# mit-han-lab/duo-attention

Measured on NVIDIA H100. Metric: decode tok/s @512K ctx (+ prefill tok/s @128K in `prefill`), Llama-3-8B, DuoAttention 50% retrieval heads, higher is better.
Workload: dtype bf16

## Files before the change

duo_attention_b200/csrc/attn_tc.cu:

```cuda
#include <cstdlib>

#include "duo_common.cuh"

namespace duo {

constexpr int TC_THREADS = 384;
constexpr int TC_TILE = 128;
constexpr int TC_BOX_BYTES = TC_TILE * 128;
constexpr int TC_TILE_BYTES = 2 * TC_BOX_BYTES;
constexpr int TC_MAX_W = 2048;
constexpr int TC_SMEM_BYTES = 5 * TC_TILE_BYTES + TC_MAX_W + 1024;

struct TcParams {
  void* out;
  long long out_batch_stride;
  int q_len, n_q_heads, group, n_full, n_stream, batch;
  int sink, recent, W;
  long long full_len, total, lo;
  float scale_log2;
  int cache_scan;
  int n_tok_tiles;
  int seq_rank, seq_world, seq_block;
  float* part_o;
  float* part_lse;
};

__device__ __forceinline__ void wg_fence() { asm volatile("wgmma.fence.sync.aligned;" ::: "memory"); }
__device__ __forceinline__ void wg_commit() { asm volatile("wgmma.commit_group.sync.aligned;" ::: "memory"); }
template <int N>
__device__ __forceinline__ void wg_wait() {
  asm volatile("wgmma.wait_group.sync.aligned %0;" ::"n"(N) : "memory");
}
__device__ __forceinline__ void wg_fence_regs(float (&d)[64]) {
#pragma unroll
  for (int i = 0; i < 64; ++i) asm volatile("" : "+f"(d[i])::"memory");
}

__device__ __forceinline__ uint64_t make_smem_desc(uint32_t saddr, uint32_t lbo_bytes, uint32_t sbo_bytes) {
  uint64_t d = 0;
  d |= (uint64_t)((saddr >> 4) & 0x3FFF);
  d |= (uint64_t)((lbo_bytes >> 4) & 0x3FFF) << 16;
  d |= (uint64_t)((sbo_bytes >> 4) & 0x3FFF) << 32;
  d |= 1ull << 62;
  return d;
}

template <bool BF16>
__device__ __forceinline__ void wgmma_ss(float (&d)[64], uint64_t adesc, uint64_t bdesc, uint32_t accum) {
  if constexpr (BF16) {
    asm volatile(
        "{\n\t.reg .pred p;\n\tsetp.ne.b32 p, %66, 0;\n\t"
        "wgmma.mma_async.sync.aligned.m64n128k16.f32.bf16.bf16 {%0,%1,%2,%3,%4,%5,%6,%7,%8,%9,%10,%11,%12,%13,%14,%15,%16,%17,%18,%19,%20,%21,%22,%23,%24,%25,%26,%27,%28,%29,%30,%31,%32,%33,%34,%35,%36,%37,%38,%39,%40,%41,%42,%43,%44,%45,%46,%47,%48,%49,%50,%51,%52,%53,%54,%55,%56,%57,%58,%59,%60,%61,%62,%63}, %64, %65, p, 1, 1, 0, 0;\n\t}"
        : "+f"(d[0]), "+f"(d[1]), "+f"(d[2]), "+f"(d[3]), "+f"(d[4]), "+f"(d[5]), "+f"(d[6]), "+f"(d[7]), "+f"(d[8]), "+f"(d[9]), "+f"(d[10]), "+f"(d[11]), "+f"(d[12]), "+f"(d[13]), "+f"(d[14]), "+f"(d[15]), "+f"(d[16]), "+f"(d[17]), "+f"(d[18]), "+f"(d[19]), "+f"(d[20]), "+f"(d[21]), "+f"(d[22]), "+f"(d[23]), "+f"(d[24]), "+f"(d[25]), "+f"(d[26]), "+f"(d[27]), "+f"(d[28]), "+f"(d[29]), "+f"(d[30]), "+f"(d[31]), "+f"(d[32]), "+f"(d[33]), "+f"(d[34]), "+f"(d[35]), "+f"(d[36]), "+f"(d[37]), "+f"(d[38]), "+f"(d[39]), "+f"(d[40]), "+f"(d[41]), "+f"(d[42]), "+f"(d[43]), "+f"(d[44]), "+f"(d[45]), "+f"(d[46]), "+f"(d[47]), "+f"(d[48]), "+f"(d[49]), "+f"(d[50]), "+f"(d[51]), "+f"(d[52]), "+f"(d[53]), "+f"(d[54]), "+f"(d[55]), "+f"(d[56]), "+f"(d[57]), "+f"(d[58]), "+f"(d[59]), "+f"(d[60]), "+f"(d[61]), "+f"(d[62]), "+f"(d[63])
        : "l"(adesc), "l"(bdesc), "r"(accum));
  } else {
    asm volatile(
        "{\n\t.reg .pred p;\n\tsetp.ne.b32 p, %66, 0;\n\t"
        "wgmma.mma_async.sync.aligned.m64n128k16.f32.f16.f16 {%0,%1,%2,%3,%4,%5,%6,%7,%8,%9,%10,%11,%12,%13,%14,%15,%16,%17,%18,%19,%20,%21,%22,%23,%24,%25,%26,%27,%28,%29,%30,%31,%32,%33,%34,%35,%36,%37,%38,%39,%40,%41,%42,%43,%44,%45,%46,%47,%48,%49,%50,%51,%52,%53,%54,%55,%56,%57,%58,%59,%60,%61,%62,%63}, %64, %65, p, 1, 1, 0, 0;\n\t}"
        : "+f"(d[0]), "+f"(d[1]), "+f"(d[2]), "+f"(d[3]), "+f"(d[4]), "+f"(d[5]), "+f"(d[6]), "+f"(d[7]), "+f"(d[8]), "+f"(d[9]), "+f"(d[10]), "+f"(d[11]), "+f"(d[12]), "+f"(d[13]), "+f"(d[14]), "+f"(d[15]), "+f"(d[16]), "+f"(d[17]), "+f"(d[18]), "+f"(d[19]), "+f"(d[20]), "+f"(d[21]), "+f"(d[22]), "+f"(d[23]), "+f"(d[24]), "+f"(d[25]), "+f"(d[26]), "+f"(d[27]), "+f"(d[28]), "+f"(d[29]), "+f"(d[30]), "+f"(d[31]), "+f"(d[32]), "+f"(d[33]), "+f"(d[34]), "+f"(d[35]), "+f"(d[36]), "+f"(d[37]), "+f"(d[38]), "+f"(d[39]), "+f"(d[40]), "+f"(d[41]), "+f"(d[42]), "+f"(d[43]), "+f"(d[44]), "+f"(d[45]), "+f"(d[46]), "+f"(d[47]), "+f"(d[48]), "+f"(d[49]), "+f"(d[50]), "+f"(d[51]), "+f"(d[52]), "+f"(d[53]), "+f"(d[54]), "+f"(d[55]), "+f"(d[56]), "+f"(d[57]), "+f"(d[58]), "+f"(d[59]), "+f"(d[60]), "+f"(d[61]), "+f"(d[62]), "+f"(d[63])
        : "l"(adesc), "l"(bdesc), "r"(accum));
  }
}
template <bool BF16>
__device__ __forceinline__ void wgmma_rs(float (&d)[64], const uint32_t* a, uint64_t bdesc) {
  if constexpr (BF16) {
    asm volatile(
        "{\n\t.reg .pred p;\n\tsetp.ne.b32 p, %69, 0;\n\t"
        "wgmma.mma_async.sync.aligned.m64n128k16.f32.bf16.bf16 {%0,%1,%2,%3,%4,%5,%6,%7,%8,%9,%10,%11,%12,%13,%14,%15,%16,%17,%18,%19,%20,%21,%22,%23,%24,%25,%26,%27,%28,%29,%30,%31,%32,%33,%34,%35,%36,%37,%38,%39,%40,%41,%42,%43,%44,%45,%46,%47,%48,%49,%50,%51,%52,%53,%54,%55,%56,%57,%58,%59,%60,%61,%62,%63}, {%64, %65, %66, %67}, %68, p, 1, 1, 1;\n\t}"
        : "+f"(d[0]), "+f"(d[1]), "+f"(d[2]), "+f"(d[3]), "+f"(d[4]), "+f"(d[5]), "+f"(d[6]), "+f"(d[7]), "+f"(d[8]), "+f"(d[9]), "+f"(d[10]), "+f"(d[11]), "+f"(d[12]), "+f"(d[13]), "+f"(d[14]), "+f"(d[15]), "+f"(d[16]), "+f"(d[17]), "+f"(d[18]), "+f"(d[19]), "+f"(d[20]), "+f"(d[21]), "+f"(d[22]), "+f"(d[23]), "+f"(d[24]), "+f"(d[25]), "+f"(d[26]), "+f"(d[27]), "+f"(d[28]), "+f"(d[29]), "+f"(d[30]), "+f"(d[31]), "+f"(d[32]), "+f"(d[33]), "+f"(d[34]), "+f"(d[35]), "+f"(d[36]), "+f"(d[37]), "+f"(d[38]), "+f"(d[39]), "+f"(d[40]), "+f"(d[41]), "+f"(d[42]), "+f"(d[43]), "+f"(d[44]), "+f"(d[45]), "+f"(d[46]), "+f"(d[47]), "+f"(d[48]), "+f"(d[49]), "+f"(d[50]), "+f"(d[51]), "+f"(d[52]), "+f"(d[53]), "+f"(d[54]), "+f"(d[55]), "+f"(d[56]), "+f"(d[57]), "+f"(d[58]), "+f"(d[59]), "+f"(d[60]), "+f"(d[61]), "+f"(d[62]), "+f"(d[63])
        : "r"(a[0]), "r"(a[1]), "r"(a[2]), "r"(a[3]), "l"(bdesc), "r"(1));
  } else {
    asm volatile(
        "{\n\t.reg .pred p;\n\tsetp.ne.b32 p, %69, 0;\n\t"
        "wgmma.mma_async.sync.aligned.m64n128k16.f32.f16.f16 {%0,%1,%2,%3,%4,%5,%6,%7,%8,%9,%10,%11,%12,%13,%14,%15,%16,%17,%18,%19,%20,%21,%22,%23,%24,%25,%26,%27,%28,%29,%30,%31,%32,%33,%34,%35,%36,%37,%38,%39,%40,%41,%42,%43,%44,%45,%46,%47,%48,%49,%50,%51,%52,%53,%54,%55,%56,%57,%58,%59,%60,%61,%62,%63}, {%64, %65, %66, %67}, %68, p, 1, 1, 1;\n\t}"
        : "+f"(d[0]), "+f"(d[1]), "+f"(d[2]), "+f"(d[3]), "+f"(d[4]), "+f"(d[5]), "+f"(d[6]), "+f"(d[7]), "+f"(d[8]), "+f"(d[9]), "+f"(d[10]), "+f"(d[11]), "+f"(d[12]), "+f"(d[13]), "+f"(d[14]), "+f"(d[15]), "+f"(d[16]), "+f"(d[17]), "+f"(d[18]), "+f"(d[19]), "+f"(d[20]), "+f"(d[21]), "+f"(d[22]), "+f"(d[23]), "+f"(d[24]), "+f"(d[25]), "+f"(d[26]), "+f"(d[27]), "+f"(d[28]), "+f"(d[29]), "+f"(d[30]), "+f"(d[31]), "+f"(d[32]), "+f"(d[33]), "+f"(d[34]), "+f"(d[35]), "+f"(d[36]), "+f"(d[37]), "+f"(d[38]), "+f"(d[39]), "+f"(d[40]), "+f"(d[41]), "+f"(d[42]), "+f"(d[43]), "+f"(d[44]), "+f"(d[45]), "+f"(d[46]), "+f"(d[47]), "+f"(d[48]), "+f"(d[49]), "+f"(d[50]), "+f"(d[51]), "+f"(d[52]), "+f"(d[53]), "+f"(d[54]), "+f"(d[55]), "+f"(d[56]), "+f"(d[57]), "+f"(d[58]), "+f"(d[59]), "+f"(d[60]), "+f"(d[61]), "+f"(d[62]), "+f"(d[63])
        : "r"(a[0]), "r"(a[1]), "r"(a[2]), "r"(a[3]), "l"(bdesc), "r"(1));
  }
}

template <typename T>
struct TcType;
template <>
struct TcType<__nv_bfloat16> {
  static constexpr bool bf16 = true;
  __device__ static uint32_t pack(float a, float b) {
    __nv_bfloat162 v = __floats2bfloat162_rn(a, b);
    return *reinterpret_cast<uint32_t*>(&v);
  }
};
template <>
struct TcType<__half> {
  static constexpr bool bf16 = false;
  __device__ static uint32_t pack(float a, float b) {
    __half2 v = __floats2half2_rn(a, b);
    return *reinterpret_cast<uint32_t*>(&v);
  }
};

struct TcBarriers {
  uint64_t q_full;
  uint64_t k_full[2], k_empty[2], v_full[2], v_empty[2];
};

template <typename T, bool SEQ = false, bool SHARE = false>
__global__ void __launch_bounds__(TC_THREADS, 1)
duo_attn_tc_kernel(const __grid_constant__ CUtensorMap map_q, const __grid_constant__ CUtensorMap map_fk,
                   const __grid_constant__ CUtensorMap map_fv, const __grid_constant__ CUtensorMap map_rk,
                   const __grid_constant__ CUtensorMap map_rv, const TcParams p,
                   const __grid_constant__ CUtensorMap map_pk, const __grid_constant__ CUtensorMap map_pv,
                   const long long share_len) {
  static_assert(!(SEQ && SHARE), "a shared prefix is not sequence-sharded");
  extern __shared__ __align__(1024) uint8_t smem_raw[];
  uint8_t* smem = reinterpret_cast<uint8_t*>((reinterpret_cast<uintptr_t>(smem_raw) + 1023) & ~uintptr_t(1023));
  __shared__ TcBarriers bars;

  uint8_t* sQ = smem;
  uint8_t* sK = smem + 1 * TC_TILE_BYTES;
  uint8_t* sV = smem + 3 * TC_TILE_BYTES;
  uint8_t* sValid = smem + 5 * TC_TILE_BYTES;

  const int tid = threadIdx.x;
  const int b = blockIdx.y;

  int x = blockIdx.x;
  const int per_kvh = p.group * p.n_tok_tiles;
  const int kvh = x / per_kvh;
  x -= kvh * per_kvh;
  const int qh = kvh * p.group + x / p.n_tok_tiles;
  const int tok0 = (p.n_tok_tiles - 1 - (x % p.n_tok_tiles)) * TC_TILE;
  const bool is_full = kvh < p.n_full;
  const int tok_hi = min(p.q_len, tok0 + TC_TILE);
  long long a0 = 0, a1, b0 = 0, b1 = 0, base;
  if (is_full) {
    base = p.full_len;
    a1 = p.full_len + tok_hi;
    if constexpr (SEQ) a1 = seq_local_len(a1, p.seq_rank, p.seq_world, p.seq_block);
  } else {
    base = p.W;
    a1 = p.cache_scan;
    b0 = p.W;
    b1 = (long long)p.W + tok_hi;
  }
  const int nA = (int)((a1 - a0 + TC_TILE - 1) / TC_TILE);
  const int nB = (int)((b1 - b0 + TC_TILE - 1) / TC_TILE);
  const int n_tiles = nA + nB;
  const CUtensorMap* mk = is_full ? &map_fk : &map_rk;
  const CUtensorMap* mv = is_full ? &map_fv : &map_rv;
  const int head_coord = is_full ? (b * p.n_full + kvh) : (b * p.n_stream + (kvh - p.n_full));
  auto tile_start = [&](int i) -> long long {
    return i < nA ? a0 + (long long)i * TC_TILE : b0 + (long long)(i - nA) * TC_TILE;
  };

  if (tid == 0) {
    prefetch_tmap(&map_q);
    prefetch_tmap(mk);
    prefetch_tmap(mv);
    if constexpr (SHARE) {
      if (is_full) {
        prefetch_tmap(&map_pk);
        prefetch_tmap(&map_pv);
      }
    }
    mbar_init(&bars.q_full, 1);
    for (int s = 0; s < 2; ++s) {
      mbar_init(&bars.k_full[s], 1);
      mbar_init(&bars.k_empty[s], 256);
      mbar_init(&bars.v_full[s], 1);
      mbar_init(&bars.v_empty[s], 256);
    }
    fence_barrier_init();
  }
  if (!is_full) {
    for (int j = tid; j < p.W; j += TC_THREADS) sValid[j] = stream_slot_valid(j, p.sink, p.recent, p.total, p.lo) ? 1 : 0;
  }
  __syncthreads();

  if (tid < 128) {
    asm volatile("setmaxnreg.dec.sync.aligned.u32 24;");
    if constexpr (SEQ) {
      if (n_tiles == 0) return;
    }
    if (tid == 0) {
      mbar_expect_tx(&bars.q_full, TC_TILE_BYTES);
      tma_load_3d(sQ, &map_q, &bars.q_full, qh * kHeadDim, tok0, b);
      tma_load_3d(sQ + TC_BOX_BYTES, &map_q, &bars.q_full, qh * kHeadDim + 64, tok0, b);
      for (int j = 0; j < n_tiles; ++j) {
        const int st = j & 1;
        const uint32_t ph = (j >> 1) & 1;
        if constexpr (SHARE) {
          const long long t0 = tile_start(j);
          const bool pre = is_full && t0 < share_len;
          const CUtensorMap* tk = pre ? &map_pk : mk;
          const CUtensorMap* tv = pre ? &map_pv : mv;
          const int r0 = (int)(is_full && !pre ? t0 - share_len : t0);
          mbar_wait(&bars.k_empty[st], ph ^ 1);
          mbar_expect_tx(&bars.k_full[st], TC_TILE_BYTES);
          tma_load_3d(sK + st * TC_TILE_BYTES, tk, &bars.k_full[st], 0, r0, head_coord);
          tma_load_3d(sK + st * TC_TILE_BYTES + TC_BOX_BYTES, tk, &bars.k_full[st], 64, r0, head_coord);
          mbar_wait(&bars.v_empty[st], ph ^ 1);
          mbar_expect_tx(&bars.v_full[st], TC_TILE_BYTES);
          tma_load_3d(sV + st * TC_TILE_BYTES, tv, &bars.v_full[st], 0, r0, head_coord);
          tma_load_3d(sV + st * TC_TILE_BYTES + TC_BOX_BYTES, tv, &bars.v_full[st], 64, r0, head_coord);
          continue;
        }
        const int j0 = (int)tile_start(j);
        mbar_wait(&bars.k_empty[st], ph ^ 1);
        mbar_expect_tx(&bars.k_full[st], TC_TILE_BYTES);
        tma_load_3d(sK + st * TC_TILE_BYTES, mk, &bars.k_full[st], 0, j0, head_coord);
        tma_load_3d(sK + st * TC_TILE_BYTES + TC_BOX_BYTES, mk, &bars.k_full[st], 64, j0, head_coord);
        mbar_wait(&bars.v_empty[st], ph ^ 1);
        mbar_expect_tx(&bars.v_full[st], TC_TILE_BYTES);
        tma_load_3d(sV + st * TC_TILE_BYTES, mv, &bars.v_full[st], 0, j0, head_coord);
        tma_load_3d(sV + st * TC_TILE_BYTES + TC_BOX_BYTES, mv, &bars.v_full[st], 64, j0, head_coord);
      }
    }
    return;
  }

  asm volatile("setmaxnreg.inc.sync.aligned.u32 240;");
  constexpr bool kBf16 = TcType<T>::bf16;
  const int wg = (tid >> 7) - 1;
  const int wt = tid & 127;
  const int quad = wt & 3;
  const int row0 = wg * 64 + (wt >> 5) * 16 + ((wt & 31) >> 2);
  const float c = p.scale_log2;
  long long min_limit = base + tok0 + wg * 64;
  int tok[2];
  bool row_ok[2];
  long long limit[2];
#pragma unroll
  for (int i = 0; i < 2; ++i) {
    tok[i] = tok0 + row0 + 8 * i;
    row_ok[i] = tok[i] < p.q_len;
    limit[i] = base + tok[i];
  }
  auto seq_last_key = [&](int t) { return seq_local_len(p.full_len + t + 1, p.seq_rank, p.seq_world, p.seq_block) - 1; };
  if constexpr (SEQ) {
    if (is_full) {
      min_limit = seq_last_key(tok0 + wg * 64);
#pragma unroll
      for (int i = 0; i < 2; ++i) limit[i] = seq_last_key(tok[i]);
    }
  }

  const uint32_t q_addr = smem_u32(sQ) + wg * 64 * 128, k_addr = smem_u32(sK), v_addr = smem_u32(sV);
  auto issue_s = [&](float (&s)[64], int st) {
    const uint32_t ka = k_addr + st * TC_TILE_BYTES;
#pragma unroll
    for (int kk = 0; kk < 8; ++kk) {
      const uint32_t off = (kk >> 2) * TC_BOX_BYTES + (kk & 3) * 32;
      wgmma_ss<kBf16>(s, make_smem_desc(q_addr + off, 16, 1024), make_smem_desc(ka + off, 16, 1024), kk > 0);
    }
  };
  auto issue_pv = [&](float (&o)[64], const uint32_t (&pk)[32], int st) {
    const uint32_t va = v_addr + st * TC_TILE_BYTES;
#pragma unroll
    for (int kk = 0; kk < 8; ++kk) wgmma_rs<kBf16>(o, &pk[4 * kk], make_smem_desc(va + kk * 2048, TC_BOX_BYTES, 1024));
  };

  float s[64], o[64];
#pragma unroll
  for (int i = 0; i < 64; ++i) o[i] = 0.f;
  float m_run[2] = {-INFINITY, -INFINITY};
  float l_run[2] = {0.f, 0.f};

  auto store_partial = [&](int i, float inv, float l) {
    if (!row_ok[i]) return;
    const long long row = ((long long)b * p.q_len + tok[i]) * p.n_q_heads + qh;
#pragma unroll
    for (int nb = 0; nb < 16; ++nb)
      *reinterpret_cast<float2*>(p.part_o + row * kHeadDim + nb * 8 + quad * 2) =
          make_float2(o[nb * 4 + 2 * i] * inv, o[nb * 4 + 2 * i + 1] * inv);
    if (quad == 0) p.part_lse[row] = l > 0.f ? m_run[i] * c + log2f(l) : -INFINITY;
  };
  if constexpr (SEQ) {
    if (n_tiles == 0) {
      store_partial(0, 0.f, 0.f);
      store_partial(1, 0.f, 0.f);
      return;
    }
  }
  mbar_wait(&bars.q_full, 0);
  mbar_wait(&bars.k_full[0], 0);
  wg_fence();
  issue_s(s, 0);
  wg_commit();
  wg_wait<0>();
  wg_fence_regs(s);
  mbar_arrive(&bars.k_empty[0]);

  for (int j = 0; j < n_tiles; ++j) {
    const int st = j & 1;
    const uint32_t ph = (j >> 1) & 1;
    const long long j0 = tile_start(j);
    const long long jend = (j < nA) ? a1 : b1;
    const bool cache_seg = (!is_full) && (j < nA);
    const bool need_mask = cache_seg || (j0 + TC_TILE > jend) || (j0 + TC_TILE - 1 > min_limit);
    if (need_mask) {
#pragma unroll
      for (int nb = 0; nb < 16; ++nb) {
#pragma unroll
        for (int e = 0; e < 2; ++e) {
          const long long jj = j0 + nb * 8 + quad * 2 + e;
          bool slot_ok = jj < jend;
          if (cache_seg) slot_ok = slot_ok && (jj < p.W) && (sValid[jj < p.W ? jj : 0] != 0);
#pragma unroll
          for (int i = 0; i < 2; ++i)
            if (!(slot_ok && row_ok[i] && jj <= limit[i])) s[nb * 4 + 2 * i + e] = -INFINITY;
        }
      }
    }
    uint32_t pk[32];
#pragma unroll
    for (int i = 0; i < 2; ++i) {
      float mx = -INFINITY;
#pragma unroll
      for (int nb = 0; nb < 16; ++nb) mx = fmaxf(mx, fmaxf(s[nb * 4 + 2 * i], s[nb * 4 + 2 * i + 1]));
      mx = fmaxf(mx, __shfl_xor_sync(0xffffffffu, mx, 1));
      mx = fmaxf(mx, __shfl_xor_sync(0xffffffffu, mx, 2));
      const float m_new = fmaxf(m_run[i], mx);
      const float alpha = (m_new == -INFINITY) ? 1.f : fast_exp2((m_run[i] - m_new) * c);
      const float mref_c = (m_new == -INFINITY) ? 0.f : m_new * c;
      m_run[i] = m_new;
      float rs = 0.f;
#pragma unroll
      for (int nb = 0; nb < 16; ++nb) {
        const float p0 = fast_exp2(__fmaf_rn(s[nb * 4 + 2 * i], c, -mref_c));
        const float p1 = fast_exp2(__fmaf_rn(s[nb * 4 + 2 * i + 1], c, -mref_c));
        rs += p0 + p1;
        pk[nb * 2 + i] = TcType<T>::pack(p0, p1);
        o[nb * 4 + 2 * i] *= alpha;
        o[nb * 4 + 2 * i + 1] *= alpha;
      }
      l_run[i] = l_run[i] * alpha + rs;
    }
    mbar_wait_spin(&bars.v_full[st], ph);
    wg_fence();
    issue_pv(o, pk, st);
    wg_commit();
    const bool more = j + 1 < n_tiles;
    if (more) {
      const int st1 = (j + 1) & 1;
      mbar_wait_spin(&bars.k_full[st1], ((j + 1) >> 1) & 1);
      wg_fence();
      issue_s(s, st1);
      wg_commit();
    }
    wg_wait<0>();
    wg_fence_regs(o);
    wg_fence_regs(s);
    mbar_arrive(&bars.v_empty[st]);
    if (more) mbar_arrive(&bars.k_empty[(j + 1) & 1]);
  }

  if constexpr (SEQ) {
    if (is_full) {
#pragma unroll
      for (int i = 0; i < 2; ++i) {
        float l = l_run[i];
        l += __shfl_xor_sync(0xffffffffu, l, 1);
        l += __shfl_xor_sync(0xffffffffu, l, 2);
        store_partial(i, l > 0.f ? 1.f / l : 0.f, l);
      }
      return;
    }
  }
  T* out_b = reinterpret_cast<T*>(p.out) + (long long)b * p.out_batch_stride;
#pragma unroll
  for (int i = 0; i < 2; ++i) {
    float l = l_run[i];
    l += __shfl_xor_sync(0xffffffffu, l, 1);
    l += __shfl_xor_sync(0xffffffffu, l, 2);
    const float inv = l > 0.f ? 1.f / l : 0.f;
    if (row_ok[i]) {
      T* dst = out_b + ((long long)tok[i] * p.n_q_heads + qh) * kHeadDim + quad * 2;
#pragma unroll
      for (int nb = 0; nb < 16; ++nb)
        *reinterpret_cast<uint32_t*>(dst + nb * 8) = TcType<T>::pack(o[nb * 4 + 2 * i] * inv, o[nb * 4 + 2 * i + 1] * inv);
    }
  }
}

typedef CUresult (*EncodeTiledFn)(CUtensorMap*, CUtensorMapDataType, cuuint32_t, void*, const cuuint64_t*,
                                  const cuuint64_t*, const cuuint32_t*, const cuuint32_t*, CUtensorMapInterleave,
                                  CUtensorMapSwizzle, CUtensorMapL2promotion, CUtensorMapFloatOOBfill);
EncodeTiledFn get_encode_fn();

bool tc_prefill_supported(const duo_layer* L, const duo_cache_state* st, int q_len) {
  (void)st;
  if (L->d.kv_format != DUO_KV_SAME) return false;
  if (q_len < TC_TILE) return false;
  if (L->d.sink + L->d.recent > TC_MAX_W) return false;
  return true;
}

template <bool SEQ, bool SHARE = false>
static int launch_tc(const duo_layer* L, const duo_cache_state* st, const void* q, long long q_row_stride, void* out,
                     float* part_o, float* part_lse, int q_len, float scale, cudaStream_t stream,
                     const duo_layer* prefix = nullptr, long long share_len = 0) {
  const duo_layer_desc& d = L->d;
  EncodeTiledFn fn = get_encode_fn();
  if (!fn) return DUO_ECUDA;
  CUtensorMap map_q;
  {
    cuuint64_t dims[3] = {(cuuint64_t)q_row_stride, (cuuint64_t)q_len, (cuuint64_t)d.batch};
    cuuint64_t strides[2] = {(cuuint64_t)q_row_stride * 2, (cuuint64_t)q_row_stride * 2 * (cuuint64_t)q_len};
    cuuint32_t box[3] = {64, TC_TILE, 1};
    cuuint32_t estr[3] = {1, 1, 1};
    CUresult r = fn(&map_q, d.dtype == DUO_DT_BF16 ? CU_TENSOR_MAP_DATA_TYPE_BFLOAT16 : CU_TENSOR_MAP_DATA_TYPE_FLOAT16, 3,
                    const_cast<void*>(q), dims, strides, box, estr, CU_TENSOR_MAP_INTERLEAVE_NONE,
                    CU_TENSOR_MAP_SWIZZLE_128B, CU_TENSOR_MAP_L2_PROMOTION_L2_256B, CU_TENSOR_MAP_FLOAT_OOB_FILL_NONE);
    if (r != CUDA_SUCCESS) {
      set_error("cuTensorMapEncodeTiled(q) failed with CUresult %d", (int)r);
      return DUO_ECUDA;
    }
  }
  TcParams p{};
  p.out = out;
  const int n_q = (d.n_full + d.n_stream) * d.group;
  p.out_batch_stride = (long long)q_len * n_q * kHeadDim;
  p.q_len = q_len;
  p.n_q_heads = n_q;
  p.group = d.group;
  p.n_full = d.n_full;
  p.n_stream = d.n_stream;
  p.batch = d.batch;
  p.sink = d.sink;
  p.recent = d.recent;
  p.W = d.sink + d.recent;
  p.full_len = st->full_len;
  p.total = st->total;
  p.lo = st->lo;
  p.scale_log2 = scale * 1.4426950408889634f;
  p.cache_scan = (int)std::min<long long>(p.W, st->total);
  p.n_tok_tiles = (q_len + TC_TILE - 1) / TC_TILE;
  p.seq_rank = st->seq_rank;
  p.seq_world = st->seq_world;
  p.seq_block = st->seq_block;
  p.part_o = part_o;
  p.part_lse = part_lse;
  const dim3 grid(n_q * p.n_tok_tiles, d.batch);
  const KvMaps m = kv_maps(L, true);
  const KvMaps pm = kv_maps(SHARE ? prefix : L, true);
  return dispatch_dtype(d.dtype, [&](auto t) {
    auto kern = duo_attn_tc_kernel<decltype(t), SEQ, SHARE>;
    static unsigned long long attr_mask = 0;
    if (int rc = ensure_dyn_smem(kern, TC_SMEM_BYTES, &attr_mask)) return rc;
    kern<<<grid, TC_THREADS, TC_SMEM_BYTES, stream>>>(map_q, *m.fk, *m.fv, *m.rk, *m.rv, p, *pm.fk, *pm.fv, share_len);
    DUO_CUDA_TRY(cudaGetLastError());
    return DUO_OK;
  });
}

int launch_attn_tc(const duo_layer* L, const duo_cache_state* st, const void* q, long long q_row_stride, void* out,
                   int q_len, float scale, cudaStream_t stream) {
  return launch_tc<false>(L, st, q, q_row_stride, out, nullptr, nullptr, q_len, scale, stream);
}

int launch_attn_tc_seq(const duo_layer* L, const duo_cache_state* st, const void* q, long long q_row_stride, void* out,
                       float* part_o, float* part_lse, int q_len, float scale, cudaStream_t stream) {
  return launch_tc<true>(L, st, q, q_row_stride, out, part_o, part_lse, q_len, scale, stream);
}

int launch_attn_tc_shared(const duo_layer* L, const duo_layer* prefix, long long share_len, const duo_cache_state* st,
                          const void* q, long long q_row_stride, void* out, int q_len, float scale, cudaStream_t stream) {
  return launch_tc<false, true>(L, st, q, q_row_stride, out, nullptr, nullptr, q_len, scale, stream, prefix, share_len);
}

}
```

Measured before the change: 56.56.

## Overlap next-tile QK^T with softmax and add ping-pong warpgroup scheduling

Restructures the wgmma attention main loop FA3-style. Each iteration issues S for tile j and PV for tile j-1 together, then runs softmax for tile j while the PV is still in flight, applying the rescale to O afterwards. Named barriers make the two consumer warpgroups take turns issuing tensor-core work, so one group's softmax can hide behind the other's MMAs. This costs extra live registers (packed P kept across iterations) and adds barrier coordination that could deadlock if the turn counts mismatch.

```diff
diff --git a/duo_attention_b200/csrc/attn_tc.cu b/duo_attention_b200/csrc/attn_tc.cu
--- a/duo_attention_b200/csrc/attn_tc.cu
+++ b/duo_attention_b200/csrc/attn_tc.cu
@@ -34,6 +34,18 @@
 __device__ __forceinline__ void wg_fence_regs(float (&d)[64]) {
 #pragma unroll
   for (int i = 0; i < 64; ++i) asm volatile("" : "+f"(d[i])::"memory");
+}
+__device__ __forceinline__ void wg_fence_regs(uint32_t (&a)[32]) {
+#pragma unroll
+  for (int i = 0; i < 32; ++i) asm volatile("" : "+r"(a[i])::"memory");
+}
+template <int ID>
+__device__ __forceinline__ void wg_pair_sync() {
+  asm volatile("bar.sync %0, 256;" ::"n"(ID) : "memory");
+}
+template <int ID>
+__device__ __forceinline__ void wg_pair_arrive() {
+  asm volatile("bar.arrive %0, 256;" ::"n"(ID) : "memory");
 }
 
 __device__ __forceinline__ uint64_t make_smem_desc(uint32_t saddr, uint32_t lbo_bytes, uint32_t sbo_bytes) {
@@ -280,18 +292,7 @@
       return;
     }
   }
-  mbar_wait(&bars.q_full, 0);
-  mbar_wait(&bars.k_full[0], 0);
-  wg_fence();
-  issue_s(s, 0);
-  wg_commit();
-  wg_wait<0>();
-  wg_fence_regs(s);
-  mbar_arrive(&bars.k_empty[0]);
-
-  for (int j = 0; j < n_tiles; ++j) {
-    const int st = j & 1;
-    const uint32_t ph = (j >> 1) & 1;
+  auto softmax_tile = [&](int j, float (&alpha)[2]) {
     const long long j0 = tile_start(j);
     const long long jend = (j < nA) ? a1 : b1;
     const bool cache_seg = (!is_full) && (j < nA);
@@ -310,7 +311,6 @@
         }
       }
     }
-    uint32_t pk[32];
 #pragma unroll
     for (int i = 0; i < 2; ++i) {
       float mx = -INFINITY;
@@ -319,38 +319,89 @@
       mx = fmaxf(mx, __shfl_xor_sync(0xffffffffu, mx, 1));
       mx = fmaxf(mx, __shfl_xor_sync(0xffffffffu, mx, 2));
       const float m_new = fmaxf(m_run[i], mx);
-      const float alpha = (m_new == -INFINITY) ? 1.f : fast_exp2((m_run[i] - m_new) * c);
+      alpha[i] = (m_new == -INFINITY) ? 1.f : fast_exp2((m_run[i] - m_new) * c);
       const float mref_c = (m_new == -INFINITY) ? 0.f : m_new * c;
       m_run[i] = m_new;
       float rs = 0.f;
 #pragma unroll
       for (int nb = 0; nb < 16; ++nb) {
-        const float p0 = fast_exp2(__fmaf_rn(s[nb * 4 + 2 * i], c, -mref_c));
-        const float p1 = fast_exp2(__fmaf_rn(s[nb * 4 + 2 * i + 1], c, -mref_c));
-        rs += p0 + p1;
-        pk[nb * 2 + i] = TcType<T>::pack(p0, p1);
-        o[nb * 4 + 2 * i] *= alpha;
-        o[nb * 4 + 2 * i + 1] *= alpha;
+        s[nb * 4 + 2 * i] = fast_exp2(__fmaf_rn(s[nb * 4 + 2 * i], c, -mref_c));
+        s[nb * 4 + 2 * i + 1] = fast_exp2(__fmaf_rn(s[nb * 4 + 2 * i + 1], c, -mref_c));
+        rs += s[nb * 4 + 2 * i] + s[nb * 4 + 2 * i + 1];
       }
-      l_run[i] = l_run[i] * alpha + rs;
-    }
-    mbar_wait_spin(&bars.v_full[st], ph);
+      l_run[i] = l_run[i] * alpha[i] + rs;
+    }
+  };
+  uint32_t pk[32];
+  auto pack_p = [&] {
+#pragma unroll
+    for (int nb = 0; nb < 16; ++nb)
+#pragma unroll
+      for (int i = 0; i < 2; ++i) pk[nb * 2 + i] = TcType<T>::pack(s[nb * 4 + 2 * i], s[nb * 4 + 2 * i + 1]);
+  };
+
+  auto turn_begin = [&] {
+    if (wg == 0) wg_pair_sync<1>();
+    else wg_pair_sync<2>();
+  };
+  auto turn_end = [&](bool last) {
+    if (wg == 0) wg_pair_arrive<2>();
+    else if (!last) wg_pair_arrive<1>();
+  };
+  float alpha[2];
+  if (wg == 1) wg_pair_arrive<1>();
+  mbar_wait(&bars.q_full, 0);
+  mbar_wait(&bars.k_full[0], 0);
+  turn_begin();
+  wg_fence();
+  issue_s(s, 0);
+  wg_commit();
+  turn_end(false);
+  wg_wait<0>();
+  wg_fence_regs(s);
+  mbar_arrive(&bars.k_empty[0]);
+  softmax_tile(0, alpha);
+  pack_p();
+
+  for (int j = 1; j < n_tiles; ++j) {
+    const int st = j & 1, stp = st ^ 1;
+    mbar_wait_spin(&bars.k_full[st], (j >> 1) & 1);
+    mbar_wait_spin(&bars.v_full[stp], ((j - 1) >> 1) & 1);
+    turn_begin();
+    wg_fence();
+    issue_s(s, st);
+    wg_commit();
+    issue_pv(o, pk, stp);
+    wg_commit();
+    turn_end(false);
+    wg_wait<1>();
+    wg_fence_regs(s);
+    mbar_arrive(&bars.k_empty[st]);
+    softmax_tile(j, alpha);
+    wg_wait<0>();
+    wg_fence_regs(o);
+    wg_fence_regs(pk);
+    mbar_arrive(&bars.v_empty[stp]);
+#pragma unroll
+    for (int nb = 0; nb < 16; ++nb)
+#pragma unroll
+      for (int i = 0; i < 2; ++i) {
+        o[nb * 4 + 2 * i] *= alpha[i];
+        o[nb * 4 + 2 * i + 1] *= alpha[i];
+      }
+    pack_p();
+  }
+  {
+    const int st = (n_tiles - 1) & 1;
+    mbar_wait_spin(&bars.v_full[st], ((n_tiles - 1) >> 1) & 1);
+    turn_begin();
     wg_fence();
     issue_pv(o, pk, st);
     wg_commit();
-    const bool more = j + 1 < n_tiles;
-    if (more) {
-      const int st1 = (j + 1) & 1;
-      mbar_wait_spin(&bars.k_full[st1], ((j + 1) >> 1) & 1);
-      wg_fence();
-      issue_s(s, st1);
-      wg_commit();
-    }
+    turn_end(true);
     wg_wait<0>();
     wg_fence_regs(o);
-    wg_fence_regs(s);
     mbar_arrive(&bars.v_empty[st]);
-    if (more) mbar_arrive(&bars.k_empty[(j + 1) & 1]);
   }
 
   if constexpr (SEQ) {
```

After: 56.54 (median of 6 runs). About the same (-0.0%).
